# simplew4y/VeritasFi

Hardware: AMD Instinct MI355X
Metric: queries/sec top-100 over 10Mx768 corpus (higher is better)
Workload: dtype f16

## Files before the change

veritasfi_amd/build.py:

```python
from __future__ import annotations

import os
import shutil
import subprocess
import sys

HERE = os.path.dirname(os.path.abspath(__file__))
CSRC = os.path.join(HERE, "csrc")
LIBDIR = os.path.join(HERE, "lib")
LIB = os.path.join(LIBDIR, os.environ.get("VF_BUILD_LIB", "libveritasfi_hip.so"))
SOURCES = ["vf_kernels.hip", "vf_api.hip", "vf_transformer.hip", "vf_sparse.hip"]
HEADERS = ["vf_internal.h", os.path.join("..", "..", "include", "veritasfi_hip.h"), "vf_ksplit_geom.h"]
ARCH = "gfx950"
FLAGS = ["-O3", "-std=c++17", "-fPIC", f"--offload-arch={ARCH}", "-Wall", "-Wno-unused-function"]
EXTRA = os.environ.get("VF_BUILD_FLAGS", "").split()


def _hipcc() -> str:
    for cand in (shutil.which("hipcc"), "/opt/rocm/bin/hipcc"):
        if cand and os.path.exists(cand):
            return cand
    raise RuntimeError("hipcc not found: the HIP library cannot be built (no fallback exists)")


def _stale(target: str, deps) -> bool:
    if not os.path.exists(target):
        return True
# ... 71 lines not shown
```

veritasfi_amd/csrc/vf_kernels.hip:

```cpp
#include "vf_internal.h"

#include <float.h>
#include <algorithm>
#include <type_traits>

#include <mutex>

namespace vf {

typedef _Float16 h8 __attribute__((ext_vector_type(8)));
typedef _Float16 h4 __attribute__((ext_vector_type(4)));
typedef float f16v __attribute__((ext_vector_type(16)));
typedef int i4v __attribute__((ext_vector_type(4)));
typedef int i16v __attribute__((ext_vector_type(16)));
typedef int i8v __attribute__((ext_vector_type(8)));

__device__ __forceinline__ float group16_tree(float acc) {
    acc = acc + __shfl_down(acc, 8, 16);
    acc = acc + __shfl_down(acc, 4, 16);
    acc = acc + __shfl_down(acc, 2, 16);
    acc = acc + __shfl_down(acc, 1, 16);
    return acc;
}

// ... 14 lines not shown
    if (e == 15u && m == 7u) return (unsigned short)(sign | 0x7E00u);
    return (unsigned short)(sign | ((e + 8u) << 10) | (m << 7));
}

__device__ __forceinline__ float e4m3_to_float(u32 b) {
    return (float)__builtin_bit_cast(_Float16, e4m3_to_f16_bits(b));
}

__device__ __forceinline__ float load_elem(const void* rows, int dt, long long idx) {
    if (dt == VF_DTYPE_F16) return (float)((const _Float16*)rows)[idx];
    if (dt == VF_DTYPE_FP8_E4M3) return e4m3_to_float(((const unsigned char*)rows)[idx]);
    if (dt == VF_DTYPE_INT8) return (float)((int)((const unsigned char*)rows)[idx] - 128);
    return ((const float*)rows)[idx];
}

__device__ __forceinline__ float bin_x(float s) { return __builtin_fmaf(s, 0.5f * kHistBins, 0.5f * kHistBins); }
__device__ __forceinline__ int bin_of_x(float x) {
    int b = (int)floorf(x);
    return b < 0 ? 0 : (b > kHistBins - 1 ? kHistBins - 1 : b);
}

__device__ __forceinline__ int next_pow2(int n) {
    int p = 1;
    while (p < n) p <<= 1;
    return p;
}

__global__ __launch_bounds__(256) void k_prep_rows(const void* rows, int dt, long long n, int d, int dp,
                                                    void* scan, float* norm, float* inv_scan) {
    const int l = threadIdx.x & 15;
    const long long r = (long long)blockIdx.x * 16 + (threadIdx.x >> 4);
    if (r >= n) return;
    const long long base = r * (long long)d;
    float acc = 0.0f, mx = 0.0f;
    for (int j = l; j < d; j += 16) {
// ... 777 lines not shown
        static_assert(INV_LDS, "the offsets ride in the scratch half the inverse norms' DMA fills");
#pragma unroll
        for (int g = 0; g < 4; ++g) {
            const float4 v = *(const float4*)(e.inv_lds + 128 + (8 * g + 4 * h) * 4);
            off16[4 * g] = v.x; off16[4 * g + 1] = v.y; off16[4 * g + 2] = v.z; off16[4 * g + 3] = v.w;
        }
    }
    const long long left = hi - t0;
    const int lf = __builtin_amdgcn_readfirstlane((int)(left < kRowTile ? left : kRowTile));
    if (lf < kRowTile) {
#pragma unroll
        for (int reg = 0; reg < 16; ++reg) inv16[reg] = ((reg & 3) + 8 * (reg >> 2) + 4 * h) < lf ? inv16[reg] : __builtin_nanf("");
    }
    typedef float mvec __attribute__((ext_vector_type(NT * 16)));
    mvec m;
    float tb[NT];
    bool any = false;
#pragma unroll
    for (int nt = 0; nt < NT; ++nt) {
        const int q = nt * kQueryTile + r31;
        const int t = tau_lds[q];
        tb[nt] = q < a.nq ? (t <= 0 ? -INFINITY : (float)t) : INFINITY;
        float top = -INFINITY;
#pragma unroll
        for (int reg = 0; reg < 16; ++reg) {
            if constexpr (OFF) m[nt * 16 + reg] = acc[nt][reg] * inv16[reg] + off16[reg];
            else m[nt * 16 + reg] = acc[nt][reg] * inv16[reg];
            top = fmaxf(top, m[nt * 16 + reg]);
        }
        any |= bin_x(top) >= tb[nt];
    }
    if (__ballot(any) == 0ull) return;
    u32 mask = 0;
#pragma unroll
    for (int nt = 0; nt < NT; ++nt)
#pragma unroll
        for (int reg = 0; reg < 16; ++reg) mask |= (bin_x(m[nt * 16 + reg]) >= tb[nt]) ? (1u << (nt * 16 + reg)) : 0u;
    const unsigned long long hot = __ballot(mask != 0u);
    if (hot == 0ull) return;
    if (a.debug & 4) return;
    u32 umask = 0u, total = 0u;
    if (__popcll(hot) <= 8) {
        for (unsigned long long hb = hot; hb != 0ull; hb &= hb - 1ull) {
            const u32 m = (u32)__builtin_amdgcn_readlane((int)mask, __builtin_ctzll(hb));
            umask |= m;
            total += (u32)__popc(m);
        }
    } else {
        umask = wave_or_u32(mask);
        total = wave_sum_u32((u32)__popc(mask));
    }
    u32* stage_cnt = (u32*)ctl;
// ... 6 lines not shown
    const bool need = (base >> rs) != ((base + total) >> rs);
    if (a.debug & 8) return;
    u32 run = base;
    const u32 edge = (((base + total) >> rs) << rs) - 1u;
    int qq = 0;
    for (u32 um = umask; um != 0u; um &= um - 1u) {
        const int pair = __builtin_ctz(um);
        const int nt = pair >> 4, reg = pair & 15;
        const int q = nt * kQueryTile + r31;
        const bool mine = ((mask >> pair) & 1u) != 0u;
        const unsigned long long bal = __ballot(mine);
        if (mine) {
            const u32 slot = run + __builtin_amdgcn_mbcnt_hi((u32)(bal >> 32), __builtin_amdgcn_mbcnt_lo((u32)bal, 0u));
            const int rr = (reg & 3) + 8 * (reg >> 2) + 4 * h;
            const float sc = m[pair];
            const u32 bin = (u32)bin_of_x(bin_x(sc));
            const u32 key = orderkey(sc), row = (u32)(t0 + rr);
            if (slot < (u32)a.stage_cap) {
                stage_ent[slot] = make_uint4(row, key, (u32)q | (bin << 8), 1u);
            } else {
                const u32 gs = atomicAdd(a.cnt + q * kCntStride, 1u);
                if (gs < (u32)a.cap) a.cand[(long long)q * a.cap + gs] = ((u64)key << 32) | (u64)row;
                atomicAdd(a.hist + (long long)q * kHistBins + bin, 1u);
                atomicAdd(a.hist_coarse + q * 64 + (bin >> 5), 1u);
            }
        }
        const u32 nxt = run + (u32)__popcll(bal);
        if (run <= edge && edge < nxt) qq = nt * kQueryTile + ((__ffsll((long long)bal) - 1) & 31);
        run = nxt;
    }
    if (a.debug & 2) return;
    if constexpr (!PUBLISH) return;
    if (need) {
        const int nb = wave_tau_two_level(a.hist_coarse + qq * 64, a.hist + (long long)qq * kHistBins, a.kprime, lane) - (a.band_q ? a.band_q[qq] : a.tau_band);
        if (lane == 0 && nb > 0) {
            atomicMax(a.tau_bin + qq, nb);
            atomicMax(tau_lds + qq, nb);
        }
        for (u32 blk = base >> rs; blk < (base + total) >> rs; ++blk)
        for (u32 j = (u32)lane; j < R; j += 64u) {
            const u32 idx = (blk << rs) + j;
            if (idx >= (u32)a.stage_cap) break;
            const uint4 en = stage_ent[idx];
            if (en.w == 1u) {
                const u32 q = en.z & 0xFFu, bin = en.z >> 8;
                if (q < (u32)QN_of<NT>() && bin < (u32)kHistBins) {
                    atomicAdd(a.hist + (long long)q * kHistBins + bin, 1u);
                    atomicAdd(a.hist_coarse + q * 64 + (bin >> 5), 1u);
                }
            }
        }
    }
}

#define VF_ISSUE(BUF, ...)                                                        \
    do {                                                                          \
        if constexpr (F8 != 0) issue_loads_f8<G>(BUF, __VA_ARGS__);               \
        else issue_loads<G>(BUF, __VA_ARGS__);                                    \
    } while (0)
#define VF_COMPUTE(ACC, BUF, ...)                                                 \
    do {                                                                          \
// ... 185 lines not shown
            const u32 q = e.z & 0xFFu;
            if (e.w != 1u || q >= (u32)QN) continue;
            ent[i].w = 2u + atomicAdd(qcnt + q, 1u);
        }
        __syncthreads();
        if (tid < QN) {
            const u32 c = qcnt[tid];
            qbase[tid] = c ? atomicAdd(a.cnt + tid * kCntStride, c) : 0u;
        }
        __syncthreads();
        for (u32 i = tid; i < nst; i += kScanThreads) {
            const uint4 e = ent[i];
            if (e.w < 2u) continue;
            const u32 q = e.z & 0xFFu;
            const u32 gs = qbase[q] + (e.w - 2u);
            if (gs < (u32)a.cap) a.cand[(long long)q * a.cap + gs] = ((u64)e.y << 32) | (u64)e.x;
        }
        if (dbg) dbg[3] = wall_clock64();
    }
}

template <int MODE, int P, int D>
__global__ __launch_bounds__(kKsThreads) void k_scan_ksplit(ScanArgs a) {
    static_assert(P >= kKsRegSegs && P <= 16 && P % D == 0, "segments per wave: 10..16, ring depth divides it");
    extern __shared__ __attribute__((aligned(16))) char smem[];
    constexpr int XS = P - kKsRegSegs;
    const int tid = threadIdx.x;
    const int lane = tid & 63, wid = __builtin_amdgcn_readfirstlane(tid >> 6);
    const int r31 = lane & 31, h = lane >> 5;
    const int S = ks_segs(a.dp);
    const int sbeg = ks_seg_begin(S, wid), send = ks_seg_begin(S, wid + 1);
// ... 105 lines not shown
            const u32 q = e.z & 0xFFu;
            if (e.w != 1u || q >= (u32)kQueryTile) continue;
            ent[i].w = 2u + atomicAdd(qcnt + q, 1u);
        }
        __syncthreads();
        if (tid < kQueryTile) {
            const u32 c = qcnt[tid];
            qbase[tid] = c ? atomicAdd(a.cnt + tid * kCntStride, c) : 0u;
        }
        __syncthreads();
        for (u32 i = tid; i < nst; i += kKsThreads) {
            const uint4 e = ent[i];
            if (e.w < 2u) continue;
            const u32 q = e.z & 0xFFu;
            const u32 gs = qbase[q] + (e.w - 2u);
            if (gs < (u32)a.cap) a.cand[(long long)q * a.cap + gs] = ((u64)e.y << 32) | (u64)e.x;
        }
    }
}

static_assert(kKs8CtlBytes == kCtlBytes, "vf_ksplit_geom.h budgets the control block the scans use");

__device__ __forceinline__ void ks_flush(const ScanArgs& a, char* ctl, char* red, int tid) {
    __syncthreads();
    const u32 staged = *(const u32*)ctl;
    const u32 nst = staged < (u32)a.stage_cap ? staged : (u32)a.stage_cap;
    uint4* ent = (uint4*)(ctl + kCtlBytes);
    u32* qcnt = (u32*)red;
    u32* qbase = qcnt + kQueryTile;
    if (tid < kQueryTile) qcnt[tid] = 0u;
    __syncthreads();
// ... 2 lines not shown
        const u32 q = e.z & 0xFFu;
        if (e.w != 1u || q >= (u32)kQueryTile) continue;
        ent[i].w = 2u + atomicAdd(qcnt + q, 1u);
    }
    __syncthreads();
    if (tid < kQueryTile) {
        const u32 c = qcnt[tid];
        qbase[tid] = c ? atomicAdd(a.cnt + tid * kCntStride, c) : 0u;
    }
    __syncthreads();
    for (u32 i = tid; i < nst; i += kKsThreads) {
        const uint4 e = ent[i];
        if (e.w < 2u) continue;
        const u32 q = e.z & 0xFFu;
        const u32 gs = qbase[q] + (e.w - 2u);
        if (gs < (u32)a.cap) a.cand[(long long)q * a.cap + gs] = ((u64)e.y << 32) | (u64)e.x;
    }
}

template <int MODE, int P>
__global__ __launch_bounds__(kKsThreads) void k_scan_ksplit8(ScanArgs a) {
    static_assert(P >= kKs8RegSegs && P <= kKs8MaxSegs, "segments per wave: 5..8");
    extern __shared__ __attribute__((aligned(16))) char smem[];
    constexpr int XS = P - kKs8RegSegs;
    const int tid = threadIdx.x;
    const int lane = tid & 63, wid = __builtin_amdgcn_readfirstlane(tid >> 6);
    const int r31 = lane & 31, h = lane >> 5;
    const int S = ks8_segs(a.dp);
    const int sbeg = ks8_seg_begin(S, wid), send = ks8_seg_begin(S, wid + 1);
    const bool has_last = sbeg + P - 1 < send;
    const long long swg = (long long)a.samp * kKsSampWaves;
// ... 141 lines not shown
    int* tau_lds = (int*)(ctl + 16);
    const uint4* stage_ent = (const uint4*)(ctl + kCtlBytes);
    const u32 R = (u32)a.refresh_every;
    u32 done_blk = 0;
    for (;;) {
        const u32 fin = *waves_done;
        const u32 staged = *stage_cnt;
        const u32 avail = staged < (u32)a.stage_cap ? staged : (u32)a.stage_cap;
        const u32 ready = fin == (u32)kScan2Waves ? avail / R : (avail >= R / 2 ? (avail - R / 2) / R : 0u);
        if (done_blk < ready) {
            const u32 blk = done_blk++;
            int qq = -1;
            for (u32 j = (u32)lane; j < R; j += 64u) {
                const uint4 en = stage_ent[blk * R + j];
                if (en.w == 1u) {
                    const u32 q = en.z & 0xFFu, bin = en.z >> 8;
                    if (q < (u32)QN && bin < (u32)kHistBins) {
                        atomicAdd(a.hist + (long long)q * kHistBins + bin, 1u);
                        atomicAdd(a.hist_coarse + q * 64 + (bin >> 5), 1u);
                        if (j == R - 1) qq = (int)q;
                    }
                }
            }
#pragma unroll
            for (int o = 32; o; o >>= 1) qq = max(qq, __shfl_xor(qq, o));
            if (qq >= 0 && !(a.debug & 2)) {
                const int nb = wave_tau_two_level(a.hist_coarse + qq * 64, a.hist + (long long)qq * kHistBins, a.kprime, lane) - a.tau_band;
                if (lane == 0 && nb > 0) { atomicMax(a.tau_bin + qq, nb); atomicMax(tau_lds + qq, nb); }
            }
            continue;
        }
        if (fin == (u32)kScan2Waves) break;
// ... 10 lines not shown
    const unsigned long long t_entry = (a.debug & 512) ? wall_clock64() : 0ull;
    extern __shared__ __attribute__((aligned(1024))) char smem[];
    constexpr int QN = NT * kQueryTile;
    constexpr int MODE = kModeMain;
    const int tid = threadIdx.x, lane = tid & 63, wid = tid >> 6;
    const int r31 = lane & 31, h = lane >> 5;
    const long long grid = gridDim.x;
    const long long swg = (long long)a.samp * (kScanThreads / 64);
    long long range_v = blockIdx.x;
#ifdef VF_EXPERIMENTS
    if ((a.debug & 32) && a.sib) {
        unsigned hw_id, xcc_id;
        asm volatile("s_getreg_b32 %0, hwreg(HW_REG_HW_ID)\n\ts_getreg_b32 %1, hwreg(HW_REG_XCC_ID)" : "=s"(hw_id), "=s"(xcc_id));
        const unsigned key = (xcc_id & 0x7u) * 128u + ((hw_id >> 13) & 3u) * 32u + ((hw_id >> 12) & 1u) * 16u + ((hw_id >> 8) & 0xFu);
        const unsigned seen = __hip_atomic_load(a.sib + key, __ATOMIC_RELAXED, __HIP_MEMORY_SCOPE_AGENT);
        if (seen != 0xFFFFFFFFu && seen < (unsigned)grid) range_v = seen;
        else if (threadIdx.x == 0) __hip_atomic_store(a.sib + key, (unsigned)blockIdx.x, __ATOMIC_RELAXED, __HIP_MEMORY_SCOPE_AGENT);
    }
#endif
    const long long Ra = a.n * range_v / grid, Rb = a.n * (range_v + 1) / grid;
    const long long lo = (Ra + swg < Rb) ? Ra + swg : Rb, hi = Rb;
    const int ntiles = (int)((hi - lo + kRowTile - 1) / kRowTile);
    const int S = a.dp >> (F8 ? 7 : 6);
    char* ring = smem + (size_t)wid * (kRing * kSegBytes);
    char* img = smem + kScan2Waves * kRing * kSegBytes;
    char* scratch = img + (size_t)a.dp * QN * 2 + (size_t)wid * kScratchBytes;
    char* ctl = img + (size_t)a.dp * QN * 2 + kScan2Waves * kScratchBytes;
    u32* next_tile = (u32*)(ctl + 4);
    const unsigned ring_l = (unsigned)__builtin_amdgcn_readfirstlane((int)lds_addr(ring)), scratch_l = (unsigned)__builtin_amdgcn_readfirstlane((int)lds_addr(scratch));

    const int drow = lane >> 3;
    struct TileSrc { unsigned long long ua; unsigned v[4]; };
    auto src_of = [&](int tile) -> TileSrc {
        const long long t0_ = lo + (long long)tile * kRowTile;
        TileSrc ts;
        ts.ua = (unsigned long long)(a.rows + t0_ * a.row_bytes);
        ts.ua = ((unsigned long long)(unsigned)__builtin_amdgcn_readfirstlane((int)(ts.ua >> 32)) << 32) | (unsigned)__builtin_amdgcn_readfirstlane((int)ts.ua);
#pragma unroll
        for (int m = 0; m < 4; ++m) {
            const int row = 8 * m + drow;
            long long r = t0_ + row;
            r = r < hi - 1 ? r : hi - 1;
            ts.v[m] = (unsigned)((r - t0_) * a.row_bytes) + ((((lane & 7) ^ ((row >> 1) & 7))) << 4);
        }
        return ts;
    };
    auto issue_seg = [&](const TileSrc& src, int seg, int buf) {
        dma16x4(src.ua + (unsigned long long)seg * 128ull, src.v[0], src.v[1], src.v[2], src.v[3], ring_l + buf * kSegBytes);
    };
    auto issue_epi = [&](long long t0, bool sync_tau, int par) {
        par = __builtin_amdgcn_readfirstlane(par);
        dma4(a.inv_scan + t0 + r31, scratch_l + par * 512 + 256);
        if (sync_tau) dma4(a.tau_bin + (lane < QN ? lane : QN - 1), scratch_l + par * 512);
    };

    const bool service = kScan2Service && wid == kScan2Waves;
    int cur_tile = __builtin_amdgcn_readfirstlane(wid);
    bool active = !service && cur_tile < ntiles;
    TileSrc src_cur{}, src_nxt{};
    if (active) {
        src_cur = src_of(cur_tile);
        issue_epi(lo + (long long)cur_tile * kRowTile, !kScan2Service, 0);
        for (int sg = 0; sg < kRing; ++sg) issue_seg(src_cur, sg, sg);
    }
    {
        const char* srcq = (const char*)a.qimg;
        const int nkb = ((a.dp >> 3) * QN) >> 6;
        const unsigned img_l = (unsigned)__builtin_amdgcn_readfirstlane((int)lds_addr(img));
        const int wu = __builtin_amdgcn_readfirstlane(wid);
        if (wu < kScan2Waves)
            for (int c = wu; c < nkb; c += kScan2Waves) dma16(srcq + ((long long)c << 10) + (lane << 4), img_l + ((unsigned)c << 10));
        asm volatile("s_waitcnt vmcnt(0)" ::: "memory");
        uint4* z = (uint4*)ctl;
        const int nz = kCtlBytes / 16 + a.stage_cap;
        for (int i = tid; i < nz; i += kScan2Threads) z[i] = make_uint4(0u, (i == 0) ? (u32)kScan2Waves : 0u, 0u, 0u);
    }
// ... 14 lines not shown
        dbg[70] = ((unsigned long long)xcc_id << 32) | hw_id;
    }
    if (service) k_scan2_service<NT>(a, ctl, lane);
#ifdef VF_EXPERIMENTS
    const int passes = (a.debug & 64) ? 2 : 1;
#else
    constexpr int passes = 1;
#endif
    int tiles_done = 0;
    for (int pass = 0; pass < passes; ++pass) {
    if (pass > 0) {
        asm volatile("s_waitcnt vmcnt(0)" ::: "memory");
        __syncthreads();
        if (tid == 0) *next_tile = (u32)kScan2Waves;
        __syncthreads();
        cur_tile = wid;
        if (active) {
            src_cur = src_of(cur_tile);
            issue_epi(lo + (long long)cur_tile * kRowTile, !kScan2Service, tiles_done & 1);
#pragma unroll
            for (int sg = 0; sg < kRing; ++sg) issue_seg(src_cur, sg, sg);
        }
    }
    if (active) {
        f16v acc[NT];
#pragma unroll
        for (int nt = 0; nt < NT; ++nt)
#pragma unroll
            for (int e = 0; e < 16; ++e) acc[nt][e] = 0.0f;
        int buf = 0;
        while (true) {
            const long long t0 = lo + (long long)cur_tile * kRowTile;
            int claimed;
            {
                int v_ = 0;
                if (lane == 0) v_ = (int)atomicAdd(next_tile, 1u);
                claimed = __builtin_amdgcn_readfirstlane(v_);
            }
            const bool more = claimed < ntiles;
            const int nxt = more ? claimed : cur_tile;
            src_nxt = src_of(nxt);
            const bool sync_now = !kScan2Service && (tiles_done & (kScan2Waves - 1)) == wid;
            const bool sync_next = !kScan2Service && ((tiles_done + 1) & (kScan2Waves - 1)) == wid;
            if (dbg && dbg_rec > 4 && tiles_done < 64) dbg[4 + tiles_done] = wall_clock64();
            for (int sg = 0; sg < S; ++sg) {
                asm volatile("s_waitcnt vmcnt(8)" ::: "memory");
                const char* ab = a_lane + buf * kSegBytes;
                if constexpr (F8 == 0) {
                    const char* bb = lds_lane + (long long)sg * (8 * QN * 16);
#pragma unroll
                    for (int i = 0; i < 4; ++i) {
                        const h8 af = *(const h8*)(ab + (((4 * h + i) ^ asw) << 4));
#pragma unroll
                        for (int nt = 0; nt < NT; ++nt) {
                            const h8 bf = *(const h8*)(bb + i * (QN * 16) + nt * (kQueryTile * 16));
                            acc[nt] = __builtin_amdgcn_mfma_f32_32x32x16_f16(af, bf, acc[nt], 0, 0, 0);
// ... 31 lines not shown
            epi.inv_lane = *(const float*)(sc + 256 + r31 * 4);
            epi.inv_lds = sc + 256;
            epi.sync_tau = sync_now;
            if (sync_now) {
#pragma unroll
                for (int nt = 0; nt < NT; ++nt) epi.tau_g[nt] = *(const int*)(sc + (nt * kQueryTile + r31) * 4);
            }
            tile_epilogue<NT, MODE, !kScan2Service, true>(a, acc, epi, t0, hi, 0, lane, ctl);
#pragma unroll
            for (int nt = 0; nt < NT; ++nt)
#pragma unroll
                for (int e = 0; e < 16; ++e) acc[nt][e] = 0.0f;
            ++tiles_done;
            if (!more) break;
            cur_tile = nxt;
            src_cur = src_nxt;
        }
    }
    }
    if (dbg && dbg_rec > 4) dbg[69] = (unsigned long long)tiles_done;
    asm volatile("s_waitcnt vmcnt(0)" ::: "memory");
    if (!service && lane == 0) atomicAdd((u32*)(ctl + 8), 1u);
    if (dbg) dbg[1] = wall_clock64();
    __syncthreads();
    if (dbg) dbg[2] = wall_clock64();
    {
        const u32 staged = *(const u32*)ctl;
        const u32 nst = staged < (u32)a.stage_cap ? staged : (u32)a.stage_cap;
        uint4* ent = (uint4*)(ctl + kCtlBytes);
        u32* qcnt = (u32*)img;
        u32* qbase = qcnt + QN;
// ... 4 lines not shown
            const u32 q = e.z & 0xFFu;
            if (e.w != 1u || q >= (u32)QN) continue;
            ent[i].w = 2u + atomicAdd(qcnt + q, 1u);
        }
        __syncthreads();
        if (tid < QN) {
            const u32 c = qcnt[tid];
            qbase[tid] = c ? atomicAdd(a.cnt + tid * kCntStride, c) : 0u;
        }
        __syncthreads();
        for (u32 i = tid; i < nst; i += kScan2Threads) {
            const uint4 e = ent[i];
            if (e.w < 2u) continue;
            const u32 q = e.z & 0xFFu;
            const u32 gs = qbase[q] + (e.w - 2u);
            if (gs < (u32)a.cap) a.cand[(long long)q * a.cap + gs] = ((u64)e.y << 32) | (u64)e.x;
        }
    }
    if (dbg) dbg[3] = wall_clock64();
}

struct Scan2rShape { int S, RB, RING; };
static Scan2rShape scan2r_shape(int dp, int f8) {
    if (!f8 && dp == 768) return {12, 6, 6};
    if (!f8 && dp == 1024) return {16, 6, 4};
    if (!f8 && dp == 512) return {8, 4, 6};
    if (!f8 && dp == 384) return {6, 3, 6};
    if (f8 == 3) return dp == 768 ? Scan2rShape{6, 6, 6} : Scan2rShape{0, 0, 0};
    if (f8 == 4) return dp == 768 ? Scan2rShape{6, 3, 6} : Scan2rShape{0, 0, 0};
    if (f8 && dp == 768) return {6, 3, 6};
    if (f8 && dp == 1024) return {8, 3, 4};
// ... 17 lines not shown
__global__ __launch_bounds__(kScan2Waves * 64) void k_scan2r(ScanArgs a) {
    const unsigned long long t_entry = (a.debug & 512) ? wall_clock64() : 0ull;
    const unsigned long long c_entry = (a.debug & 512) ? __builtin_amdgcn_s_memtime() : 0ull;
    extern __shared__ __attribute__((aligned(1024))) char smem[];
    constexpr int QN = NT * kQueryTile, THREADS = kScan2Waves * 64;
    constexpr bool I8 = F8 >= 3;
    constexpr int PLANES = F8 == 4 ? 2 : 1;
    constexpr int J = I8 ? 4 * PLANES : F8 ? 8 : 4;
    constexpr int SEGIMG = J * 2 * QN * 16;
    auto frag_off = [](int j) { return I8 ? (2 * (j & 3) * PLANES + (j >> 2)) * (QN * 16) : F8 ? ((j >> 2) * 8 + (j & 3)) * (QN * 16) : j * (QN * 16); };
    static_assert(F8 != 3 || RB == S, "the single int8 plane lives in registers whole: no LDS part");
    static_assert(S >= RING && RB <= S && RB <= 6, "ring fill and the spelled-out register segments");
    const int tid = threadIdx.x, lane = tid & 63, wid = tid >> 6;
    const int r31 = lane & 31, h = lane >> 5;
    const long long grid = (MODE == kModeSample && a.scan_grid > 0) ? a.scan_grid : gridDim.x;
    const long long swg = (long long)a.samp * (kScanThreads / 64);
    const int tps = (int)((swg + kRowTile - 1) / kRowTile);
    long long lo = 0, hi = 0;
    int ntiles;
    if (MODE == kModeSample) {
        const long long mine = (grid - (long long)blockIdx.x + gridDim.x - 1) / gridDim.x;
        ntiles = (int)(mine > 0 ? mine : 0) * tps;
    } else {
        const long long Ra = a.n * blockIdx.x / grid, Rb = a.n * (blockIdx.x + 1) / grid;
        lo = (Ra + swg < Rb) ? Ra + swg : Rb; hi = Rb;
        ntiles = (int)((hi - lo + kRowTile - 1) / kRowTile);
    }
    auto tile_rows = [&](int tile, long long& t0, long long& thi, long long& sbase) {
        if (MODE == kModeSample) {
            const int m = tile / tps, j = tile - m * tps;
            long long v = (long long)blockIdx.x + (long long)m * gridDim.x;
            v = v < grid ? v : grid - 1;
            const long long Ra = a.n * v / grid, Rb = a.n * (v + 1) / grid;
            thi = (Ra + swg < Rb) ? Ra + swg : Rb;
            t0 = Ra + (long long)j * kRowTile;
            sbase = v * swg + (long long)j * kRowTile;
        } else {
            t0 = lo + (long long)tile * kRowTile; thi = hi; sbase = 0;
        }
    };
    h8 breg[RB][J][NT];
    {
        const char* qb = (const char*)a.qimg + ((long long)((I8 ? PLANES : 4) * h) * QN + r31) * 16;
#pragma unroll
        for (int sg = 0; sg < RB; ++sg)
#pragma unroll
            for (int j = 0; j < J; ++j)
#pragma unroll
                for (int nt = 0; nt < NT; ++nt)
                    breg[sg][j][nt] = *(const h8*)(qb + (long long)sg * SEGIMG + frag_off(j) + nt * (kQueryTile * 16));
    }
    float sq[NT];
#pragma unroll
    for (int nt = 0; nt < NT; ++nt) sq[nt] = I8 ? a.q_scale[nt * kQueryTile + r31] : 1.0f;
    char* ring = smem + (size_t)wid * (RING * kSegBytes);
    char* img = smem + kScan2Waves * RING * kSegBytes;
    constexpr size_t kImgBytes = (size_t)(S - RB) * SEGIMG;
    char* scratch = img + kImgBytes + (size_t)wid * kScratchBytes;
    char* ctl = img + kImgBytes + kScan2Waves * kScratchBytes;
    u32* next_tile = (u32*)(ctl + 4);
    const unsigned ring_l = (unsigned)__builtin_amdgcn_readfirstlane((int)lds_addr(ring)), scratch_l = (unsigned)__builtin_amdgcn_readfirstlane((int)lds_addr(scratch));
    const int drow = lane >> 3;
    struct TileSrc { unsigned long long ua; unsigned v[4]; };
    auto src_of = [&](int tile) -> TileSrc {
        long long t0_, thi_, sb_;
        tile_rows(tile, t0_, thi_, sb_);
        TileSrc ts;
        const long long last_row = thi_ - 1 > 0 ? thi_ - 1 : 0;
        long long base_row = t0_ > 0 ? t0_ : 0;
        base_row = base_row < last_row ? base_row : last_row;
        ts.ua = (unsigned long long)(a.rows + base_row * a.row_bytes);
        ts.ua = ((unsigned long long)(unsigned)__builtin_amdgcn_readfirstlane((int)(ts.ua >> 32)) << 32) | (unsigned)__builtin_amdgcn_readfirstlane((int)ts.ua);
#pragma unroll
        for (int m = 0; m < 4; ++m) {
            const int row = 8 * m + drow;
            long long r = t0_ + row;
            r = r < last_row ? r : last_row;
            r = r > base_row ? r : base_row;
            ts.v[m] = (unsigned)((r - base_row) * a.row_bytes) + ((((lane & 7) ^ ((row >> 1) & 7))) << 4);
        }
        return ts;
    };
    auto first_row = [&](int tile) {
        long long t0_, thi_, sb_;
        tile_rows(tile, t0_, thi_, sb_);
        const long long last_row = thi_ - 1 > 0 ? thi_ - 1 : 0;
        return t0_ < last_row ? t0_ : last_row;
    };
    auto issue_seg = [&](const TileSrc& src, int seg, int buf) {
        dma16x4(src.ua + (unsigned long long)seg * 128ull, src.v[0], src.v[1], src.v[2], src.v[3], ring_l + buf * kSegBytes);
    };
    auto issue_epi = [&](long long t0, bool sync_tau, int par) {
        par = __builtin_amdgcn_readfirstlane(par);
        dma4((F8 >= 2 && h) ? a.off_scan + t0 + r31 : a.inv_scan + t0 + r31, scratch_l + par * 512 + 256);
        if (sync_tau) dma4(a.tau_bin + (lane < QN ? lane : QN - 1), scratch_l + par * 512);
    };
    int cur_tile = __builtin_amdgcn_readfirstlane(wid);
    const bool active = cur_tile < ntiles;
    TileSrc src_cur{}, src_nxt{};
    if (active) {
        src_cur = src_of(cur_tile);
        issue_epi(first_row(cur_tile), MODE == kModeMain, 0);
#pragma unroll
        for (int sg = 0; sg < RING; ++sg) issue_seg(src_cur, sg, sg);
    }
    typedef unsigned int u4r __attribute__((ext_vector_type(4)));
    {
        const char* srcq = (const char*)a.qimg + (long long)RB * SEGIMG;
        constexpr int nkb = (int)(kImgBytes >> 10);
        const unsigned img_l = (unsigned)__builtin_amdgcn_readfirstlane((int)lds_addr(img));
        const int wu = __builtin_amdgcn_readfirstlane(wid);
        for (int c = wu; c < nkb; c += kScan2Waves) dma16(srcq + ((long long)c << 10) + (lane << 4), img_l + ((unsigned)c << 10));
        __builtin_amdgcn_s_waitcnt(0x0F70);
        if constexpr (AR) {
#pragma unroll
            for (int sg = 0; sg < RB; ++sg)
// ... 35 lines not shown
    int tiles_done = 0;
    if (active) {
        f16v acc[NT];
        i16v acci[PLANES][NT];
#pragma unroll
        for (int nt = 0; nt < NT; ++nt)
#pragma unroll
            for (int e = 0; e < 16; ++e) {
                acc[nt][e] = 0.0f;
#pragma unroll
                for (int pl = 0; pl < PLANES; ++pl) acci[pl][nt][e] = 0;
            }
        int buf = 0;
        while (true) {
            VF_PC(pt0 = cyc())
            long long t0, t_hi, t_s0;
            tile_rows(cur_tile, t0, t_hi, t_s0);
            int claimed;
            {
                int v_ = 0;
                if (lane == 0) v_ = (int)atomicAdd(next_tile, 1u);
                claimed = __builtin_amdgcn_readfirstlane(v_);
            }
            const bool more = claimed < ntiles;
            const int nxt = more ? claimed : cur_tile;
            src_nxt = src_of(nxt);
            const bool sync_now = MODE == kModeMain && (tiles_done & (kScan2Waves - 1)) == wid;
            const bool sync_next = MODE == kModeMain && ((tiles_done + 1) & (kScan2Waves - 1)) == wid;
            if (dbg && dbg_rec > 4 && tiles_done < 64) dbg[4 + tiles_done] = wall_clock64();
            VF_PC(pt1 = cyc(); pc_head += pt1 - pt0)
            auto consume = [&](auto sg_c, const char* bb) {
                constexpr int sgc = decltype(sg_c)::value;
                VF_PC(pt0 = cyc())
                if constexpr (RING == 6) asm volatile("s_waitcnt vmcnt(20)" ::: "memory");
                else if constexpr (RING == 5) asm volatile("s_waitcnt vmcnt(16)" ::: "memory");
                else asm volatile("s_waitcnt vmcnt(12)" ::: "memory");
                static_assert(RING >= 4 && RING <= 6, "the counted waits above");
                VF_PC(pt1 = cyc(); pc_wait += pt1 - pt0; ++pc_n)
                const char* ab = a_lane + buf * kSegBytes;
                auto bfrag = [&](int j, int nt) -> h8 {
                    if constexpr (sgc >= 0) {
// ... 127 lines not shown
            }
            epi.sync_tau = sync_now;
            if (sync_now) {
#pragma unroll
                for (int nt = 0; nt < NT; ++nt) epi.tau_g[nt] = *(const int*)(sc + (nt * kQueryTile + r31) * 4);
            }
            tile_epilogue<NT, MODE, true, true, F8 >= 2>(a, acc, epi, t0, t_hi, t_s0, lane, ctl);
#pragma unroll
            for (int nt = 0; nt < NT; ++nt)
#pragma unroll
                for (int e = 0; e < 16; ++e) acc[nt][e] = 0.0f;
            VF_PC(pt1 = cyc(); pc_epi += pt1 - pt0)
            ++tiles_done;
            if (!more) break;
            cur_tile = nxt;
            src_cur = src_nxt;
        }
    }
    if (dbg && dbg_rec > 4) dbg[69] = (unsigned long long)tiles_done;
    asm volatile("s_waitcnt vmcnt(0)" ::: "memory");
    if (MODE == kModeSample) return;
    if (lane == 0) atomicAdd((u32*)(ctl + 8), 1u);
    if (dbg) dbg[1] = wall_clock64();
    __syncthreads();
    if (dbg) dbg[2] = wall_clock64();
    {
        const u32 staged = *(const u32*)ctl;
        const u32 nst = staged < (u32)a.stage_cap ? staged : (u32)a.stage_cap;
        uint4* ent = (uint4*)(ctl + kCtlBytes);
        u32* qcnt = (u32*)(kImgBytes ? img : smem);
        u32* qbase = qcnt + QN;
// ... 4 lines not shown
            const u32 q = e.z & 0xFFu;
            if (e.w != 1u || q >= (u32)QN) continue;
            ent[i].w = 2u + atomicAdd(qcnt + q, 1u);
        }
        __syncthreads();
        if (tid < QN) {
            const u32 c = qcnt[tid];
            qbase[tid] = c ? atomicAdd(a.cnt + tid * kCntStride, c) : 0u;
        }
        __syncthreads();
        for (u32 i = tid; i < nst; i += THREADS) {
            const uint4 e = ent[i];
            if (e.w < 2u) continue;
            const u32 q = e.z & 0xFFu;
            const u32 gs = qbase[q] + (e.w - 2u);
            if (gs < (u32)a.cap) a.cand[(long long)q * a.cap + gs] = ((u64)e.y << 32) | (u64)e.x;
        }
    }
    if (dbg && dbg_rec > 4) dbg[71] = __builtin_amdgcn_s_memtime() - c_entry;
#ifdef VF_EXPERIMENTS
    if (dbg && dbg_rec > 4 && prof) { dbg[4] = pc_wait; dbg[5] = pc_use; dbg[6] = pc_fill; dbg[7] = pc_head; dbg[8] = pc_epi; dbg[9] = pc_n; }
#endif
#undef VF_PC
    if (dbg) dbg[3] = wall_clock64();
}

constexpr int kWideQ = 256, kWideNT = kWideQ / kQueryTile, kWideKC = 64, kWideRows = 256;
#ifndef VF_WIDE_THREADS
#define VF_WIDE_THREADS 512
#endif
constexpr int kWideThreads = VF_WIDE_THREADS, kWideWaves = kWideThreads / 64, kWideM = kWideRows / kWideWaves / kRowTile;
// ... 1604 lines not shown
```

Baseline: 48030.

## Filter in score domain, stage raw scores, precompute full-tile DMA lane offsets

The tile epilogue now compares raw scores against a float threshold derived from the tau bin, instead of converting every score to bin space. The candidate mask is built with inline v_cmp/v_addc assembly. Staged entries store the raw float score, so the bin and orderkey are computed later, only when entries are flushed. Scan kernels also precompute per-lane DMA offsets for full tiles and skip the clamping arithmetic unless a tile is partial. Together these cut VALU work in the hot scan and epilogue, but add duplicated geometry helpers and hand-written asm whose threshold must match the old bin comparison exactly.

Result: no change. 48380 (median of 3 runs) (+0.7%).

```diff
diff --git a/veritasfi_amd/build.py b/veritasfi_amd/build.py
--- a/veritasfi_amd/build.py
+++ b/veritasfi_amd/build.py
@@ -10,7 +10,7 @@
 LIBDIR = os.path.join(HERE, "lib")
 LIB = os.path.join(LIBDIR, os.environ.get("VF_BUILD_LIB", "libveritasfi_hip.so"))
 SOURCES = ["vf_kernels.hip", "vf_api.hip", "vf_transformer.hip", "vf_sparse.hip"]
-HEADERS = ["vf_internal.h", os.path.join("..", "..", "include", "veritasfi_hip.h"), "vf_ksplit_geom.h"]
+HEADERS = ["vf_internal.h", os.path.join("..", "..", "include", "veritasfi_hip.h"), "vf_ksplit_geom.h", "vf_filter_math.h", "vf_scan2_geom.h"]
 ARCH = "gfx950"
 FLAGS = ["-O3", "-std=c++17", "-fPIC", f"--offload-arch={ARCH}", "-Wall", "-Wno-unused-function"]
 EXTRA = os.environ.get("VF_BUILD_FLAGS", "").split()
diff --git a/veritasfi_amd/csrc/vf_filter_math.h b/veritasfi_amd/csrc/vf_filter_math.h
--- /dev/null
+++ b/veritasfi_amd/csrc/vf_filter_math.h
@@ -0,0 +1,31 @@
+#pragma once
+
+#ifndef VF_HD
+#if defined(__HIPCC__)
+#define VF_HD __host__ __device__ __forceinline__
+#else
+#define VF_HD inline
+#endif
+#endif
+
+namespace vf {
+
+constexpr int kFilterBins = 2048;
+
+VF_HD float bin_x(float s) { return __builtin_fmaf(s, 0.5f * kFilterBins, 0.5f * kFilterBins); }
+VF_HD int bin_of_x(float x) {
+    int b = (int)__builtin_floorf(x);
+    return b < 0 ? 0 : (b > kFilterBins - 1 ? kFilterBins - 1 : b);
+}
+
+VF_HD float thr_of_bin(int t) {
+    const float a = (float)(t - kFilterBins / 2) * (2.0f / kFilterBins);
+    const float c = t > kFilterBins / 2 ? 0x1p-24f : (t > kFilterBins / 4 ? 0x1p-25f : 0.0f);
+    return a - c;
+}
+
+VF_HD float thr_of_tau(int t, bool real) {
+    return real ? (t <= 0 ? -__builtin_inff() : thr_of_bin(t)) : __builtin_inff();
+}
+
+}
diff --git a/veritasfi_amd/csrc/vf_kernels.hip b/veritasfi_amd/csrc/vf_kernels.hip
--- a/veritasfi_amd/csrc/vf_kernels.hip
+++ b/veritasfi_amd/csrc/vf_kernels.hip
@@ -1,4 +1,6 @@
 #include "vf_internal.h"
+#include "vf_filter_math.h"
+#include "vf_scan2_geom.h"
 
 #include <float.h>
 #include <algorithm>
@@ -52,11 +54,7 @@
     return ((const float*)rows)[idx];
 }
 
-__device__ __forceinline__ float bin_x(float s) { return __builtin_fmaf(s, 0.5f * kHistBins, 0.5f * kHistBins); }
-__device__ __forceinline__ int bin_of_x(float x) {
-    int b = (int)floorf(x);
-    return b < 0 ? 0 : (b > kHistBins - 1 ? kHistBins - 1 : b);
-}
+static_assert(kFilterBins == kHistBins, "vf_filter_math.h's bins are the threshold histogram's");
 
 __device__ __forceinline__ int next_pow2(int n) {
     int p = 1;
@@ -864,13 +862,20 @@
     }
     typedef float mvec __attribute__((ext_vector_type(NT * 16)));
     mvec m;
+    float thr[NT];
+    bool any = false;
+#ifdef VF_EXPERIMENTS
+    const bool bin_domain = (a.debug & 8192) != 0;
     float tb[NT];
-    bool any = false;
+#endif
 #pragma unroll
     for (int nt = 0; nt < NT; ++nt) {
         const int q = nt * kQueryTile + r31;
         const int t = tau_lds[q];
+        thr[nt] = thr_of_tau(t, q < a.nq);
+#ifdef VF_EXPERIMENTS
         tb[nt] = q < a.nq ? (t <= 0 ? -INFINITY : (float)t) : INFINITY;
+#endif
         float top = -INFINITY;
 #pragma unroll
         for (int reg = 0; reg < 16; ++reg) {
@@ -878,14 +883,33 @@
             else m[nt * 16 + reg] = acc[nt][reg] * inv16[reg];
             top = fmaxf(top, m[nt * 16 + reg]);
         }
-        any |= bin_x(top) >= tb[nt];
+#ifdef VF_EXPERIMENTS
+        if (bin_domain) any |= bin_x(top) >= tb[nt];
+        else
+#endif
+        any |= top >= thr[nt];
     }
     if (__ballot(any) == 0ull) return;
     u32 mask = 0;
-#pragma unroll
-    for (int nt = 0; nt < NT; ++nt)
-#pragma unroll
-        for (int reg = 0; reg < 16; ++reg) mask |= (bin_x(m[nt * 16 + reg]) >= tb[nt]) ? (1u << (nt * 16 + reg)) : 0u;
+#ifdef VF_EXPERIMENTS
+    if (bin_domain) {
+#pragma unroll
+        for (int nt = 0; nt < NT; ++nt)
+#pragma unroll
+            for (int reg = 0; reg < 16; ++reg) mask |= (bin_x(m[nt * 16 + reg]) >= tb[nt]) ? (1u << (nt * 16 + reg)) : 0u;
+    } else
+#endif
+    {
+#define VF_GE_SHIFT(N) "v_cmp_ge_f32 vcc, %" #N ", %9\n\tv_addc_co_u32 %0, vcc, %0, %0, vcc\n\t"
+#pragma unroll
+        for (int g = NT * 2 - 1; g >= 0; --g)
+            asm(VF_GE_SHIFT(1) VF_GE_SHIFT(2) VF_GE_SHIFT(3) VF_GE_SHIFT(4) VF_GE_SHIFT(5) VF_GE_SHIFT(6) VF_GE_SHIFT(7) VF_GE_SHIFT(8)
+                : "+v"(mask)
+                : "v"(m[8 * g + 7]), "v"(m[8 * g + 6]), "v"(m[8 * g + 5]), "v"(m[8 * g + 4]), "v"(m[8 * g + 3]), "v"(m[8 * g + 2]),
+                  "v"(m[8 * g + 1]), "v"(m[8 * g]), "v"(thr[g >> 1])
+                : "vcc");
+#undef VF_GE_SHIFT
+    }
     const unsigned long long hot = __ballot(mask != 0u);
     if (hot == 0ull) return;
     if (a.debug & 4) return;
@@ -922,11 +946,11 @@
             const u32 slot = run + __builtin_amdgcn_mbcnt_hi((u32)(bal >> 32), __builtin_amdgcn_mbcnt_lo((u32)bal, 0u));
             const int rr = (reg & 3) + 8 * (reg >> 2) + 4 * h;
             const float sc = m[pair];
-            const u32 bin = (u32)bin_of_x(bin_x(sc));
-            const u32 key = orderkey(sc), row = (u32)(t0 + rr);
+            const u32 row = (u32)(t0 + rr);
             if (slot < (u32)a.stage_cap) {
-                stage_ent[slot] = make_uint4(row, key, (u32)q | (bin << 8), 1u);
+                stage_ent[slot] = make_uint4(row, __float_as_uint(sc), (u32)q, 1u);
             } else {
+                const u32 bin = (u32)bin_of_x(bin_x(sc)), key = orderkey(sc);
                 const u32 gs = atomicAdd(a.cnt + q * kCntStride, 1u);
                 if (gs < (u32)a.cap) a.cand[(long long)q * a.cap + gs] = ((u64)key << 32) | (u64)row;
                 atomicAdd(a.hist + (long long)q * kHistBins + bin, 1u);
@@ -951,8 +975,8 @@
             if (idx >= (u32)a.stage_cap) break;
             const uint4 en = stage_ent[idx];
             if (en.w == 1u) {
-                const u32 q = en.z & 0xFFu, bin = en.z >> 8;
-                if (q < (u32)QN_of<NT>() && bin < (u32)kHistBins) {
+                const u32 q = en.z & 0xFFu, bin = (u32)bin_of_x(bin_x(__uint_as_float(en.y)));
+                if (q < (u32)QN_of<NT>()) {
                     atomicAdd(a.hist + (long long)q * kHistBins + bin, 1u);
                     atomicAdd(a.hist_coarse + q * 64 + (bin >> 5), 1u);
                 }
@@ -1168,7 +1192,7 @@
             if (e.w < 2u) continue;
             const u32 q = e.z & 0xFFu;
             const u32 gs = qbase[q] + (e.w - 2u);
-            if (gs < (u32)a.cap) a.cand[(long long)q * a.cap + gs] = ((u64)e.y << 32) | (u64)e.x;
+            if (gs < (u32)a.cap) a.cand[(long long)q * a.cap + gs] = ((u64)orderkey(__uint_as_float(e.y)) << 32) | (u64)e.x;
         }
         if (dbg) dbg[3] = wall_clock64();
     }
@@ -1304,7 +1328,7 @@
             if (e.w < 2u) continue;
             const u32 q = e.z & 0xFFu;
             const u32 gs = qbase[q] + (e.w - 2u);
-            if (gs < (u32)a.cap) a.cand[(long long)q * a.cap + gs] = ((u64)e.y << 32) | (u64)e.x;
+            if (gs < (u32)a.cap) a.cand[(long long)q * a.cap + gs] = ((u64)orderkey(__uint_as_float(e.y)) << 32) | (u64)e.x;
         }
     }
 }
@@ -1337,7 +1361,7 @@
         if (e.w < 2u) continue;
         const u32 q = e.z & 0xFFu;
         const u32 gs = qbase[q] + (e.w - 2u);
-        if (gs < (u32)a.cap) a.cand[(long long)q * a.cap + gs] = ((u64)e.y << 32) | (u64)e.x;
+        if (gs < (u32)a.cap) a.cand[(long long)q * a.cap + gs] = ((u64)orderkey(__uint_as_float(e.y)) << 32) | (u64)e.x;
     }
 }
 
@@ -1509,8 +1533,8 @@
             for (u32 j = (u32)lane; j < R; j += 64u) {
                 const uint4 en = stage_ent[blk * R + j];
                 if (en.w == 1u) {
-                    const u32 q = en.z & 0xFFu, bin = en.z >> 8;
-                    if (q < (u32)QN && bin < (u32)kHistBins) {
+                    const u32 q = en.z & 0xFFu, bin = (u32)bin_of_x(bin_x(__uint_as_float(en.y)));
+                    if (q < (u32)QN) {
                         atomicAdd(a.hist + (long long)q * kHistBins + bin, 1u);
                         atomicAdd(a.hist_coarse + q * 64 + (bin >> 5), 1u);
                         if (j == R - 1) qq = (int)q;
@@ -1551,7 +1575,7 @@
         asm volatile("s_getreg_b32 %0, hwreg(HW_REG_HW_ID)\n\ts_getreg_b32 %1, hwreg(HW_REG_XCC_ID)" : "=s"(hw_id), "=s"(xcc_id));
         const unsigned key = (xcc_id & 0x7u) * 128u + ((hw_id >> 13) & 3u) * 32u + ((hw_id >> 12) & 1u) * 16u + ((hw_id >> 8) & 0xFu);
         const unsigned seen = __hip_atomic_load(a.sib + key, __ATOMIC_RELAXED, __HIP_MEMORY_SCOPE_AGENT);
-        if (seen != 0xFFFFFFFFu && seen < (unsigned)grid) range_v = seen;
+        if (seen != 0xFFFFFFFFu && seen < (unsigned)grid) range_v = (unsigned)__builtin_amdgcn_readfirstlane((int)seen);
         else if (threadIdx.x == 0) __hip_atomic_store(a.sib + key, (unsigned)blockIdx.x, __ATOMIC_RELAXED, __HIP_MEMORY_SCOPE_AGENT);
     }
 #endif
@@ -1566,21 +1590,25 @@
     u32* next_tile = (u32*)(ctl + 4);
     const unsigned ring_l = (unsigned)__builtin_amdgcn_readfirstlane((int)lds_addr(ring)), scratch_l = (unsigned)__builtin_amdgcn_readfirstlane((int)lds_addr(scratch));
 
-    const int drow = lane >> 3;
-    struct TileSrc { unsigned long long ua; unsigned v[4]; };
-    auto src_of = [&](int tile) -> TileSrc {
-        const long long t0_ = lo + (long long)tile * kRowTile;
-        TileSrc ts;
-        ts.ua = (unsigned long long)(a.rows + t0_ * a.row_bytes);
+    unsigned voff_full[4];
+#pragma unroll
+    for (int m = 0; m < 4; ++m) voff_full[m] = s2_lane_off_full(lane, m, a.row_bytes);
+    struct TileSrc { unsigned long long ua; bool vfull; unsigned v[4]; };
+    auto src_of = [&](int tile, TileSrc& ts) {
+        const S2Tile t = s2_main_tile(lo, hi, tile);
+        ts.ua = (unsigned long long)(a.rows + s2_base_row(t) * a.row_bytes);
         ts.ua = ((unsigned long long)(unsigned)__builtin_amdgcn_readfirstlane((int)(ts.ua >> 32)) << 32) | (unsigned)__builtin_amdgcn_readfirstlane((int)ts.ua);
-#pragma unroll
-        for (int m = 0; m < 4; ++m) {
-            const int row = 8 * m + drow;
-            long long r = t0_ + row;
-            r = r < hi - 1 ? r : hi - 1;
-            ts.v[m] = (unsigned)((r - t0_) * a.row_bytes) + ((((lane & 7) ^ ((row >> 1) & 7))) << 4);
-        }
-        return ts;
+        if (s2_full(t)) {
+            if (!ts.vfull) {
+#pragma unroll
+                for (int m = 0; m < 4; ++m) ts.v[m] = voff_full[m];
+                ts.vfull = true;
+            }
+        } else {
+#pragma unroll
+            for (int m = 0; m < 4; ++m) ts.v[m] = s2_lane_off(t, lane, m, a.row_bytes);
+            ts.vfull = false;
+        }
     };
     auto issue_seg = [&](const TileSrc& src, int seg, int buf) {
         dma16x4(src.ua + (unsigned long long)seg * 128ull, src.v[0], src.v[1], src.v[2], src.v[3], ring_l + buf * kSegBytes);
@@ -1594,9 +1622,13 @@
     const bool service = kScan2Service && wid == kScan2Waves;
     int cur_tile = __builtin_amdgcn_readfirstlane(wid);
     bool active = !service && cur_tile < ntiles;
-    TileSrc src_cur{}, src_nxt{};
+    TileSrc src_cur, src_nxt;
+    src_cur.ua = src_nxt.ua = 0ull;
+    src_cur.vfull = src_nxt.vfull = true;
+#pragma unroll
+    for (int m = 0; m < 4; ++m) src_cur.v[m] = src_nxt.v[m] = voff_full[m];
     if (active) {
-        src_cur = src_of(cur_tile);
+        src_of(cur_tile, src_cur);
         issue_epi(lo + (long long)cur_tile * kRowTile, !kScan2Service, 0);
         for (int sg = 0; sg < kRing; ++sg) issue_seg(src_cur, sg, sg);
     }
@@ -1641,9 +1673,9 @@
         __syncthreads();
         if (tid == 0) *next_tile = (u32)kScan2Waves;
         __syncthreads();
-        cur_tile = wid;
+        cur_tile = __builtin_amdgcn_readfirstlane(wid);
         if (active) {
-            src_cur = src_of(cur_tile);
+            src_of(cur_tile, src_cur);
             issue_epi(lo + (long long)cur_tile * kRowTile, !kScan2Service, tiles_done & 1);
 #pragma unroll
             for (int sg = 0; sg < kRing; ++sg) issue_seg(src_cur, sg, sg);
@@ -1666,7 +1698,7 @@
             }
             const bool more = claimed < ntiles;
             const int nxt = more ? claimed : cur_tile;
-            src_nxt = src_of(nxt);
+            src_of(nxt, src_nxt);
             const bool sync_now = !kScan2Service && (tiles_done & (kScan2Waves - 1)) == wid;
             const bool sync_next = !kScan2Service && ((tiles_done + 1) & (kScan2Waves - 1)) == wid;
             if (dbg && dbg_rec > 4 && tiles_done < 64) dbg[4 + tiles_done] = wall_clock64();
@@ -1728,7 +1760,12 @@
             ++tiles_done;
             if (!more) break;
             cur_tile = nxt;
-            src_cur = src_nxt;
+            src_cur.ua = src_nxt.ua;
+            if (!(src_cur.vfull && src_nxt.vfull)) {
+#pragma unroll
+                for (int m = 0; m < 4; ++m) src_cur.v[m] = src_nxt.v[m];
+                src_cur.vfull = src_nxt.vfull;
+            }
         }
     }
     }
@@ -1763,7 +1800,7 @@
             if (e.w < 2u) continue;
             const u32 q = e.z & 0xFFu;
             const u32 gs = qbase[q] + (e.w - 2u);
-            if (gs < (u32)a.cap) a.cand[(long long)q * a.cap + gs] = ((u64)e.y << 32) | (u64)e.x;
+            if (gs < (u32)a.cap) a.cand[(long long)q * a.cap + gs] = ((u64)orderkey(__uint_as_float(e.y)) << 32) | (u64)e.x;
         }
     }
     if (dbg) dbg[3] = wall_clock64();
@@ -1811,30 +1848,19 @@
     const int tid = threadIdx.x, lane = tid & 63, wid = tid >> 6;
     const int r31 = lane & 31, h = lane >> 5;
     const long long grid = (MODE == kModeSample && a.scan_grid > 0) ? a.scan_grid : gridDim.x;
-    const long long swg = (long long)a.samp * (kScanThreads / 64);
-    const int tps = (int)((swg + kRowTile - 1) / kRowTile);
+    static_assert(kS2RowTile == kRowTile && kS2SampWaves == kScanThreads / 64, "vf_scan2_geom.h's tile and sample part are k_scan's");
+    const long long swg = (long long)a.samp * kS2SampWaves;
+    const int tps = s2_sample_tps(swg);
     long long lo = 0, hi = 0;
     int ntiles;
     if (MODE == kModeSample) {
-        const long long mine = (grid - (long long)blockIdx.x + gridDim.x - 1) / gridDim.x;
-        ntiles = (int)(mine > 0 ? mine : 0) * tps;
+        ntiles = s2_sample_ntiles(grid, blockIdx.x, gridDim.x, tps);
     } else {
-        const long long Ra = a.n * blockIdx.x / grid, Rb = a.n * (blockIdx.x + 1) / grid;
-        lo = (Ra + swg < Rb) ? Ra + swg : Rb; hi = Rb;
-        ntiles = (int)((hi - lo + kRowTile - 1) / kRowTile);
-    }
-    auto tile_rows = [&](int tile, long long& t0, long long& thi, long long& sbase) {
-        if (MODE == kModeSample) {
-            const int m = tile / tps, j = tile - m * tps;
-            long long v = (long long)blockIdx.x + (long long)m * gridDim.x;
-            v = v < grid ? v : grid - 1;
-            const long long Ra = a.n * v / grid, Rb = a.n * (v + 1) / grid;
-            thi = (Ra + swg < Rb) ? Ra + swg : Rb;
-            t0 = Ra + (long long)j * kRowTile;
-            sbase = v * swg + (long long)j * kRowTile;
-        } else {
-            t0 = lo + (long long)tile * kRowTile; thi = hi; sbase = 0;
-        }
+        s2_main_part(a.n, grid, blockIdx.x, swg, lo, hi);
+        ntiles = s2_main_ntiles(lo, hi);
+    }
+    auto tile_of = [&](int tile) -> S2Tile {
+        return MODE == kModeSample ? s2_sample_tile(a.n, grid, swg, tps, blockIdx.x, gridDim.x, tile) : s2_main_tile(lo, hi, tile);
     };
     h8 breg[RB][J][NT];
     {
@@ -1857,33 +1883,27 @@
     char* ctl = img + kImgBytes + kScan2Waves * kScratchBytes;
     u32* next_tile = (u32*)(ctl + 4);
     const unsigned ring_l = (unsigned)__builtin_amdgcn_readfirstlane((int)lds_addr(ring)), scratch_l = (unsigned)__builtin_amdgcn_readfirstlane((int)lds_addr(scratch));
-    const int drow = lane >> 3;
-    struct TileSrc { unsigned long long ua; unsigned v[4]; };
-    auto src_of = [&](int tile) -> TileSrc {
-        long long t0_, thi_, sb_;
-        tile_rows(tile, t0_, thi_, sb_);
-        TileSrc ts;
-        const long long last_row = thi_ - 1 > 0 ? thi_ - 1 : 0;
-        long long base_row = t0_ > 0 ? t0_ : 0;
-        base_row = base_row < last_row ? base_row : last_row;
-        ts.ua = (unsigned long long)(a.rows + base_row * a.row_bytes);
+    unsigned voff_full[4];
+#pragma unroll
+    for (int m = 0; m < 4; ++m) voff_full[m] = s2_lane_off_full(lane, m, a.row_bytes);
+    struct TileSrc { unsigned long long ua; bool vfull; unsigned v[4]; };
+    auto src_of = [&](int tile, TileSrc& ts) {
+        const S2Tile t = tile_of(tile);
+        ts.ua = (unsigned long long)(a.rows + s2_base_row(t) * a.row_bytes);
         ts.ua = ((unsigned long long)(unsigned)__builtin_amdgcn_readfirstlane((int)(ts.ua >> 32)) << 32) | (unsigned)__builtin_amdgcn_readfirstlane((int)ts.ua);
-#pragma unroll
-        for (int m = 0; m < 4; ++m) {
-            const int row = 8 * m + drow;
-            long long r = t0_ + row;
-            r = r < last_row ? r : last_row;
-            r = r > base_row ? r : base_row;
-            ts.v[m] = (unsigned)((r - base_row) * a.row_bytes) + ((((lane & 7) ^ ((row >> 1) & 7))) << 4);
-        }
-        return ts;
+        if (s2_full(t)) {
+            if (!ts.vfull) {
+#pragma unroll
+                for (int m = 0; m < 4; ++m) ts.v[m] = voff_full[m];
+                ts.vfull = true;
+            }
+        } else {
+#pragma unroll
+            for (int m = 0; m < 4; ++m) ts.v[m] = s2_lane_off(t, lane, m, a.row_bytes);
+            ts.vfull = false;
+        }
     };
-    auto first_row = [&](int tile) {
-        long long t0_, thi_, sb_;
-        tile_rows(tile, t0_, thi_, sb_);
-        const long long last_row = thi_ - 1 > 0 ? thi_ - 1 : 0;
-        return t0_ < last_row ? t0_ : last_row;
-    };
+    auto first_row = [&](int tile) { return s2_first_row(tile_of(tile)); };
     auto issue_seg = [&](const TileSrc& src, int seg, int buf) {
         dma16x4(src.ua + (unsigned long long)seg * 128ull, src.v[0], src.v[1], src.v[2], src.v[3], ring_l + buf * kSegBytes);
     };
@@ -1894,9 +1914,13 @@
     };
     int cur_tile = __builtin_amdgcn_readfirstlane(wid);
     const bool active = cur_tile < ntiles;
-    TileSrc src_cur{}, src_nxt{};
+    TileSrc src_cur, src_nxt;
+    src_cur.ua = src_nxt.ua = 0ull;
+    src_cur.vfull = src_nxt.vfull = true;
+#pragma unroll
+    for (int m = 0; m < 4; ++m) src_cur.v[m] = src_nxt.v[m] = voff_full[m];
     if (active) {
-        src_cur = src_of(cur_tile);
+        src_of(cur_tile, src_cur);
         issue_epi(first_row(cur_tile), MODE == kModeMain, 0);
 #pragma unroll
         for (int sg = 0; sg < RING; ++sg) issue_seg(src_cur, sg, sg);
@@ -1962,8 +1986,8 @@
         int buf = 0;
         while (true) {
             VF_PC(pt0 = cyc())
-            long long t0, t_hi, t_s0;
-            tile_rows(cur_tile, t0, t_hi, t_s0);
+            const S2Tile tcur = tile_of(cur_tile);
+            const long long t0 = tcur.t0, t_hi = tcur.thi, t_s0 = tcur.sbase;
             int claimed;
             {
                 int v_ = 0;
@@ -1972,7 +1996,7 @@
             }
             const bool more = claimed < ntiles;
             const int nxt = more ? claimed : cur_tile;
-            src_nxt = src_of(nxt);
+            src_of(nxt, src_nxt);
             const bool sync_now = MODE == kModeMain && (tiles_done & (kScan2Waves - 1)) == wid;
             const bool sync_next = MODE == kModeMain && ((tiles_done + 1) & (kScan2Waves - 1)) == wid;
             if (dbg && dbg_rec > 4 && tiles_done < 64) dbg[4 + tiles_done] = wall_clock64();
@@ -2130,7 +2154,12 @@
             ++tiles_done;
             if (!more) break;
             cur_tile = nxt;
-            src_cur = src_nxt;
+            src_cur.ua = src_nxt.ua;
+            if (!(src_cur.vfull && src_nxt.vfull)) {
+#pragma unroll
+                for (int m = 0; m < 4; ++m) src_cur.v[m] = src_nxt.v[m];
+                src_cur.vfull = src_nxt.vfull;
+            }
         }
     }
     if (dbg && dbg_rec > 4) dbg[69] = (unsigned long long)tiles_done;
@@ -2165,7 +2194,7 @@
             if (e.w < 2u) continue;
             const u32 q = e.z & 0xFFu;
             const u32 gs = qbase[q] + (e.w - 2u);
-            if (gs < (u32)a.cap) a.cand[(long long)q * a.cap + gs] = ((u64)e.y << 32) | (u64)e.x;
+            if (gs < (u32)a.cap) a.cand[(long long)q * a.cap + gs] = ((u64)orderkey(__uint_as_float(e.y)) << 32) | (u64)e.x;
         }
     }
     if (dbg && dbg_rec > 4) dbg[71] = __builtin_amdgcn_s_memtime() - c_entry;
diff --git a/veritasfi_amd/csrc/vf_scan2_geom.h b/veritasfi_amd/csrc/vf_scan2_geom.h
--- /dev/null
+++ b/veritasfi_amd/csrc/vf_scan2_geom.h
@@ -0,0 +1,72 @@
+#pragma once
+
+#ifndef VF_HD
+#if defined(__HIPCC__)
+#define VF_HD __host__ __device__ __forceinline__
+#else
+#define VF_HD inline
+#endif
+#endif
+
+namespace vf {
+
+constexpr int kS2RowTile = 32;
+constexpr int kS2SampWaves = 8;
+
+struct S2Tile { long long t0, thi, sbase; };
+
+VF_HD void s2_main_part(long long n, long long grid, long long v, long long swg, long long& lo, long long& hi) {
+    const long long Ra = n * v / grid, Rb = n * (v + 1) / grid;
+    lo = (Ra + swg < Rb) ? Ra + swg : Rb;
+    hi = Rb;
+}
+VF_HD int s2_main_ntiles(long long lo, long long hi) { return (int)((hi - lo + kS2RowTile - 1) / kS2RowTile); }
+VF_HD S2Tile s2_main_tile(long long lo, long long hi, int tile) {
+    S2Tile t;
+    t.t0 = lo + (long long)tile * kS2RowTile; t.thi = hi; t.sbase = 0;
+    return t;
+}
+VF_HD int s2_sample_tps(long long swg) { return (int)((swg + kS2RowTile - 1) / kS2RowTile); }
+VF_HD int s2_sample_ntiles(long long grid, long long block, long long nblocks, int tps) {
+    const long long mine = (grid - block + nblocks - 1) / nblocks;
+    return (int)(mine > 0 ? mine : 0) * tps;
+}
+VF_HD S2Tile s2_sample_tile(long long n, long long grid, long long swg, int tps, long long block, long long nblocks, int tile) {
+    const int m = tile / tps, j = tile - m * tps;
+    long long v = block + (long long)m * nblocks;
+    v = v < grid ? v : grid - 1;
+    const long long Ra = n * v / grid, Rb = n * (v + 1) / grid;
+    S2Tile t;
+    t.thi = (Ra + swg < Rb) ? Ra + swg : Rb;
+    t.t0 = Ra + (long long)j * kS2RowTile;
+    t.sbase = v * swg + (long long)j * kS2RowTile;
+    return t;
+}
+
+VF_HD bool s2_full(const S2Tile& t) { return (t.t0 | (t.thi - kS2RowTile - t.t0)) >= 0; }
+
+VF_HD long long s2_last_row(const S2Tile& t) { return t.thi - 1 > 0 ? t.thi - 1 : 0; }
+VF_HD long long s2_base_row(const S2Tile& t) {
+    const long long last_row = s2_last_row(t);
+    const long long b = t.t0 > 0 ? t.t0 : 0;
+    return b < last_row ? b : last_row;
+}
+VF_HD unsigned s2_swizzle(int lane, int row) { return (unsigned)(((lane & 7) ^ ((row >> 1) & 7)) << 4); }
+VF_HD unsigned s2_lane_off(const S2Tile& t, int lane, int m, long long row_bytes) {
+    const int row = 8 * m + (lane >> 3);
+    const long long last_row = s2_last_row(t), base_row = s2_base_row(t);
+    long long r = t.t0 + row;
+    r = r < last_row ? r : last_row;
+    r = r > base_row ? r : base_row;
+    return (unsigned)((r - base_row) * row_bytes) + s2_swizzle(lane, row);
+}
+VF_HD unsigned s2_lane_off_full(int lane, int m, long long row_bytes) {
+    const int row = 8 * m + (lane >> 3);
+    return (unsigned)((long long)row * row_bytes) + s2_swizzle(lane, row);
+}
+VF_HD long long s2_first_row(const S2Tile& t) {
+    const long long last_row = s2_last_row(t);
+    return t.t0 < last_row ? t.t0 : last_row;
+}
+
+}
```
